# sara-nl/2D-VQ-AE-2

Hardware: AMD Instinct MI355X
Metric: patches/sec (VQAE.forward: encoder -> VQ -> decoder) (higher is better)
Workload: dtype f32; 1 GPU; BASELINE configs[1] (cfg B): batch 256/GPU of 256x256x3 fp32 -> 32x32 codes, K=256, D=128, full forward; global_batch=256, parallelism=patch-sharded x1

## Files before the change

### 2d-vq-ae-2_amd/csrc/conv_wino43.hip

```cpp
#include "kernels.h"
#include "mfma.h"

namespace {

using namespace vqae;

struct W43K {
    const float* __restrict__ t1;
    const float* __restrict__ U;
    const float* __restrict__ w3;
    const float* __restrict__ w1n;
    float* xio;
    float* y2;
    const float* __restrict__ Us;
    const float* __restrict__ w3s;
    const float* __restrict__ w1ns;
    int H, M;
    float act_a, act_b, t_scale, t_b4, n_b1a, n_b1b, n_b2a, n_b2b;
};

template <int C_> struct W43Cfg {
    static constexpr int C = C_;
    static constexpr int W = C >= 128 ? 32 : 64;
    static constexpr int NT = C == 256 ? 512 : 256;
    static constexpr int NWV = NT / 64;
    static constexpr int NS = C / 32;
    static constexpr int TG = NWV / NS;
    static constexpr int TILES = 16 * TG;
    static constexpr int TC = W / 4;
    static constexpr int PXH = 4 * W;
    static constexpr int C4 = C / 4;
    static constexpr int RP = NT / C4;
    static constexpr int LDT = C + 4;
    static constexpr int KG = C / 16;
    static constexpr int KS = C / 8;
    static constexpr int NI = 2;
    static constexpr int WN = C / (32 * NI);
    static constexpr int MI = PXH / ((NWV / WN) * 32);
    static constexpr int V_BYTES = 6 * TILES * LDT * 4, T_BYTES = PXH * LDT * 4;
    static constexpr int LDS_BYTES = V_BYTES > T_BYTES ? V_BYTES : T_BYTES;
    static constexpr int LDVB = 3 * C + 8, KC = C / 32, KS2 = C / 16;
    static constexpr int VS_BYTES = 6 * TILES * LDVB * 2;
    static constexpr int LDS_SPLIT = VS_BYTES > T_BYTES ? VS_BYTES : T_BYTES;
    static_assert(TILES == 2 * TC && RP == TC && PXH / RP == 16 && MI * NI == 4, "geometry");
};
constexpr int EARLY = 1;
constexpr int RD = 4;
constexpr int NRES0 = 4;
constexpr int RT = 3;

__device__ __forceinline__ void split3(const f32x4& v, bf16x4 (&h)[3]) {
    h[0] = __builtin_convertvector(v, bf16x4);
    const f32x4 r1 = v - __builtin_convertvector(h[0], f32x4);
    h[1] = __builtin_convertvector(r1, bf16x4);
    const f32x4 r2 = r1 - __builtin_convertvector(h[1], f32x4);
    h[2] = __builtin_convertvector(r2, bf16x4);
}
__device__ __forceinline__ bf16x8 as_bf8(const f32x4& v) { return __builtin_bit_cast(bf16x8, v); }

__device__ __forceinline__ f32x4 fma4(const f32x4& a, float s, const f32x4& c) {
    return __builtin_elementwise_fma(a, f32x4{s, s, s, s}, c);
}

__device__ __forceinline__ f32x4 ldg(const float* sbase, unsigned voff_bytes) {
    return *reinterpret_cast<const f32x4*>(reinterpret_cast<const char*>(sbase) + voff_bytes);
}

template <int N> struct IC { static constexpr int value = N; };

template <int C, int TAIL, bool SPLIT>
__global__ __launch_bounds__((W43Cfg<C>::NT), (W43Cfg<C>::NT == 512 ? 1 : 2))
void wino43_trunk_kernel(const W43K p) {
    using K = W43Cfg<C>;
    constexpr int W = K::W, LDT = K::LDT, KG = K::KG, KS = K::KS, TILES = K::TILES, TC = K::TC, NS = K::NS, C4 = K::C4, RP = K::RP;
    constexpr int MI = K::MI, NI = K::NI, WN = K::WN;
    constexpr int LDVB = K::LDVB, KC = K::KC, KS2 = K::KS2;
    extern __shared__ __attribute__((aligned(16))) float lds[];
    const int tid = threadIdx.x;
    const int lane = tid & 63;
    const int wave = __builtin_amdgcn_readfirstlane(tid >> 6);
    const int li = lane & 15, q = lane >> 4;
    const int ns = wave % NS, tg = wave / NS;

    int tile_m;
    {
        const int nwg = gridDim.x, bid = blockIdx.x;
        const int qq = nwg >> 3, r = nwg & 7, xcd = bid & 7;
        tile_m = (xcd < r ? xcd * (qq + 1) : r * (qq + 1) + (xcd - r) * qq) + (bid >> 3);
    }
    const int tpi = p.H / 8;
    const int img = tile_m / tpi;
    const int row0 = 8 * (tile_m - img * tpi);
    const float* const xim = p.t1 + (int64_t)img * p.H * W * C;

    const int cg = tid % C4, tj = tid / C4;
    unsigned coff[6];
    int roff[2][6];
#pragma unroll
    for (int j = 0; j < 6; ++j) coff[j] = (unsigned)((((4 * tj - 1 + j) & (W - 1)) * C + 4 * cg) * 4);
#pragma unroll
    for (int s = 0; s < 2; ++s)
#pragma unroll
        for (int i = 0; i < 6; ++i) {
            int r = row0 + 4 * s - 1 + i;
            r = r < 0 ? r + p.H : (r >= p.H ? r - p.H : r);
            roff[s][i] = r * W * C;
        }

    f32x4 d[2][4][2];
    f32x4 w[6];
    auto issue = [&](auto kind_c, int k) __attribute__((always_inline)) {
        constexpr int KIND = decltype(kind_c)::value;
        const int s = k / 3, cp = k % 3, bf = k & 1;
#pragma unroll
        for (int i = 0; i < (KIND == 1 ? 4 : 3); ++i) {
            const int row = KIND == 0 ? 2 * i : (KIND == 5 ? 2 * i + 1 : i + 1);
#pragma unroll
            for (int jj = 0; jj < 2; ++jj) d[bf][i][jj] = ldg(xim + roff[s][row], coff[2 * cp + jj]);
        }
    };
    auto combine = [&](auto kind_c, int k, float c1, float c2, float c3) __attribute__((always_inline)) {
        constexpr int KIND = decltype(kind_c)::value;
        const int cp = k % 3, bf = k & 1;
#pragma unroll
        for (int jj = 0; jj < 2; ++jj) {
            if (KIND == 1) w[2 * cp + jj] = fma4(d[bf][0][jj], c1, fma4(d[bf][1][jj], c2, fma4(d[bf][2][jj], c3, d[bf][3][jj])));
            else w[2 * cp + jj] = fma4(d[bf][0][jj], 4.f, fma4(d[bf][1][jj], -5.f, d[bf][2][jj]));
        }
    };
    auto columns = [&](int s) __attribute__((always_inline)) {
        float* const dst = lds + (s * TC + tj) * LDT + 4 * cg;
        __bf16* const dsb = reinterpret_cast<__bf16*>(lds) + (s * TC + tj) * LDVB + 4 * cg;
        auto put = [&](int nu, const f32x4& v) __attribute__((always_inline)) {
            if constexpr (SPLIT) {
                bf16x4 h[3];
                split3(v, h);
#pragma unroll
                for (int pl = 0; pl < 3; ++pl) *reinterpret_cast<bf16x4*>(dsb + nu * TILES * LDVB + pl * C) = h[pl];
            } else {
                *reinterpret_cast<f32x4*>(dst + nu * TILES * LDT) = v;
            }
        };
        const f32x4 t1 = fma4(w[2], -4.f, w[4]), t2 = fma4(w[1], -4.f, w[3]);
        const f32x4 t3 = w[4] - w[2], t4 = w[3] - w[1];
        put(0, fma4(w[0], 4.f, fma4(w[2], -5.f, w[4])));
        put(1, t1 + t2);
        put(2, t1 - t2);
        put(3, fma4(t4, 2.f, t3));
        put(4, fma4(t4, -2.f, t3));
        put(5, fma4(w[1], 4.f, fma4(w[3], -5.f, w[5])));
    };

    const float* const ub = p.U + ns * (KG * 512);
    const float* const ubs = p.Us + ns * (KC * 1536);
    const __bf16* const vbs = reinterpret_cast<const __bf16*>(lds) + (16 * tg + li) * LDVB + 8 * q;
    const unsigned wl = 16u * lane;
    const float* const bfrag = lds + (16 * tg + li) * LDT + 4 * q;

    f32x4 Y[4][4][2];
#pragma unroll
    for (int a = 0; a < 4; ++a)
#pragma unroll
        for (int b = 0; b < 4; ++b) { Y[a][b][0] = f32x4{0.f, 0.f, 0.f, 0.f}; Y[a][b][1] = f32x4{0.f, 0.f, 0.f, 0.f}; }

    auto pass = [&](auto kind_c, auto next_c, int xi, float c1, float c2, float c3, float a1, float a2, float a3) __attribute__((always_inline)) {
        constexpr int KIND = decltype(kind_c)::value;
        constexpr int NEXT = decltype(next_c)::value;
        __builtin_amdgcn_sched_barrier(0);
#pragma unroll
        for (int j = 0; j < 6; ++j) asm volatile("" : "+v"(coff[j]));
        if (EARLY < 1) issue(kind_c, 0);
        if (EARLY < 2) issue(kind_c, 1);
#pragma unroll
        for (int k = 0; k < 6; ++k) {
            combine(kind_c, k, c1, c2, c3);
            if (k % 3 == 2) columns(k / 3);
            if (k + 2 < 6) issue(kind_c, k + 2);
        }
        __builtin_amdgcn_sched_barrier(0);
        f32x4 Z[4][2];
        f32x4 acc[2][2];
        auto fold_nu = [&](int nu) __attribute__((always_inline)) {
#pragma unroll
            for (int bl = 0; bl < 2; ++bl) {
                if (nu == 0) Z[0][bl] = Z[0][bl] + acc[0][bl];
                if (nu == 2) {
                    const f32x4 sm = acc[1][bl] + acc[0][bl], df = acc[1][bl] - acc[0][bl];
                    Z[0][bl] = Z[0][bl] + sm; Z[2][bl] = Z[2][bl] + sm;
                    Z[1][bl] = Z[1][bl] + df; Z[3][bl] = Z[3][bl] + df;
                }
                if (nu == 4) {
                    const f32x4 sm = acc[1][bl] + acc[0][bl], df = acc[1][bl] - acc[0][bl];
                    Z[0][bl] = Z[0][bl] + sm; Z[2][bl] = fma4(sm, 4.f, Z[2][bl]);
                    Z[1][bl] = fma4(df, 2.f, Z[1][bl]); Z[3][bl] = fma4(df, 8.f, Z[3][bl]);
                }
                if (nu == 5) Z[3][bl] = Z[3][bl] + acc[1][bl];
            }
            if (nu == 0 || nu == 2 || nu == 4)
                asm volatile("" : "+v"(Z[0][0]), "+v"(Z[0][1]), "+v"(Z[1][0]), "+v"(Z[1][1]), "+v"(Z[2][0]), "+v"(Z[2][1]), "+v"(Z[3][0]), "+v"(Z[3][1]));
        };
        if constexpr (SPLIT) {
            int64_t uoff = (int64_t)xi * 6 * (3 * C * C / 2);
            asm volatile("" : "+s"(uoff));
            const float* const ux = ubs + uoff;
#define WS(s, bl, pl) (((s) / KC) * (3 * C * C / 2) + 1536 * ((s) % KC) + 256 * (3 * (bl) + (pl)))
#define VB(s, pl) (*reinterpret_cast<const bf16x8*>(vbs + ((s) / KC) * TILES * LDVB + (pl) * C + 32 * ((s) % KC)))
            f32x4 w0[2][2], w1[2], w2[2];
#pragma unroll
            for (int bl = 0; bl < 2; ++bl) {
                w0[0][bl] = ldg(ux + WS(0, bl, 0), wl);
                w1[bl] = ldg(ux + WS(0, bl, 1), wl);
                w2[bl] = ldg(ux + WS(0, bl, 2), wl);
                w0[1][bl] = ldg(ux + WS(1, bl, 0), wl);
            }
            lds_barrier();
#pragma unroll
            for (int b = 0; b < 4; ++b) { Z[b][0] = f32x4{0.f, 0.f, 0.f, 0.f}; Z[b][1] = f32x4{0.f, 0.f, 0.f, 0.f}; }
            bf16x8 vb0 = VB(0, 0), vb1 = VB(0, 1), vb2 = VB(0, 2);
#pragma unroll
            for (int nu = 0; nu < 6; ++nu) {
                const int st = nu & 1;
                acc[st][0] = f32x4{0.f, 0.f, 0.f, 0.f};
                acc[st][1] = f32x4{0.f, 0.f, 0.f, 0.f};
#pragma unroll
                for (int kc = 0; kc < KC; ++kc) {
                    const int s = KC * nu + kc, sl = s & 1;
                    const bool nxt = s + 1 < 6 * KC;
#define MM(wa, vb) for (int bl = 0; bl < 2; ++bl) acc[st][bl] = __builtin_amdgcn_mfma_f32_16x16x32_bf16(as_bf8(wa[bl]), vb, acc[st][bl], 0, 0, 0)
                    MM(w1, vb1);
                    MM(w1, vb0);
                    if (nxt) for (int bl = 0; bl < 2; ++bl) w1[bl] = ldg(ux + WS(s + 1, bl, 1), wl);
                    MM(w2, vb0);
                    if (nxt) for (int bl = 0; bl < 2; ++bl) w2[bl] = ldg(ux + WS(s + 1, bl, 2), wl);
                    MM(w0[sl], vb2);
                    if (nxt) vb2 = VB(s + 1, 2);
                    MM(w0[sl], vb1);
                    if (nxt) vb1 = VB(s + 1, 1);
                    MM(w0[sl], vb0);
                    if (s + 2 < 6 * KC) for (int bl = 0; bl < 2; ++bl) w0[sl][bl] = ldg(ux + WS(s + 2, bl, 0), wl);
                    if (nxt) vb0 = VB(s + 1, 0);
#undef MM
                    __builtin_amdgcn_sched_barrier(0);
                }
                fold_nu(nu);
            }
#undef WS
#undef VB
        } else {
            int64_t uoff = (int64_t)xi * 6 * (C * C);
            asm volatile("" : "+s"(uoff));
            const float* const ux = ub + uoff;
#define WB(s) (((s) / KG) * (C * C) + 512 * ((s) % KG))
            f32x4 wq[RD][2];
#pragma unroll
            for (int s = 0; s < RD; ++s) {
                wq[s][0] = ldg(ux + WB(s), wl);
                wq[s][1] = ldg(ux + WB(s) + 256, wl);
            }
            lds_barrier();
#pragma unroll
            for (int b = 0; b < 4; ++b) { Z[b][0] = f32x4{0.f, 0.f, 0.f, 0.f}; Z[b][1] = f32x4{0.f, 0.f, 0.f, 0.f}; }
            f32x4 bq[2];
            bq[0] = *reinterpret_cast<const f32x4*>(bfrag);
#pragma unroll
            for (int nu = 0; nu < 6; ++nu) {
                const int st = nu & 1;
                acc[st][0] = f32x4{0.f, 0.f, 0.f, 0.f};
                acc[st][1] = f32x4{0.f, 0.f, 0.f, 0.f};
#pragma unroll
                for (int kg = 0; kg < KG; ++kg) {
                    const int s = KG * nu + kg;
                    if (s + 1 < 6 * KG)
                        bq[(s + 1) & 1] = *reinterpret_cast<const f32x4*>(bfrag + ((s + 1) / KG) * TILES * LDT + 16 * ((s + 1) % KG));
                    const f32x4 wa = wq[s % RD][0], wb = wq[s % RD][1];
                    if (s + RD < 6 * KG) {
                        wq[s % RD][0] = ldg(ux + WB(s + RD), wl);
                        wq[s % RD][1] = ldg(ux + WB(s + RD) + 256, wl);
                    }
#pragma unroll
                    for (int j = 0; j < 4; ++j) {
                        acc[st][0] = __builtin_amdgcn_mfma_f32_16x16x4f32(wa[j], bq[s & 1][j], acc[st][0], 0, 0, 0);
                        acc[st][1] = __builtin_amdgcn_mfma_f32_16x16x4f32(wb[j], bq[s & 1][j], acc[st][1], 0, 0, 0);
                    }
                    __builtin_amdgcn_sched_barrier(0);
                }
                fold_nu(nu);
            }
#undef WB
        }
        __builtin_amdgcn_sched_barrier(0);
        if constexpr (NEXT == 9) {
#pragma unroll
            for (int k = 0; k < EARLY; ++k)
#pragma unroll
                for (int i = 0; i < 4; ++i) {
                    const int ro = xi < 4 ? roff[0][i + 1] : roff[0][i < 3 ? 2 * i + 1 : 5];
#pragma unroll
                    for (int jj = 0; jj < 2; ++jj) d[k & 1][i][jj] = ldg(xim + ro, coff[2 * k + jj]);
                }
        } else {
            if constexpr (NEXT >= 0 && EARLY >= 1) issue(next_c, 0);
            if constexpr (NEXT >= 0 && EARLY >= 2) issue(next_c, 1);
        }
#pragma unroll
        for (int b = 0; b < 4; ++b)
#pragma unroll
            for (int bl = 0; bl < 2; ++bl) {
                if (KIND == 0) Y[0][b][bl] = Y[0][b][bl] + Z[b][bl];
                else if (KIND == 5) Y[3][b][bl] = Y[3][b][bl] + Z[b][bl];
                else {
                    Y[0][b][bl] = Y[0][b][bl] + Z[b][bl];
                    Y[1][b][bl] = fma4(Z[b][bl], a1, Y[1][b][bl]);
                    Y[2][b][bl] = fma4(Z[b][bl], a2, Y[2][b][bl]);
                    Y[3][b][bl] = fma4(Z[b][bl], a3, Y[3][b][bl]);
                }
            }
        lds_barrier();
    };

    if (EARLY >= 1) issue(IC<0>{}, 0);
    if (EARLY >= 2) issue(IC<0>{}, 1);
    pass(IC<0>{}, IC<1>{}, 0, 0.f, 0.f, 0.f, 0.f, 0.f, 0.f);
#pragma unroll 1
    for (int xi = 1; xi <= 4; ++xi) {
        const float sg = (xi & 1) ? 1.f : -1.f;
        const bool lo = xi <= 2;
        const float c1 = lo ? -4.f * sg : -2.f * sg, c2 = lo ? -4.f : -1.f, c3 = lo ? sg : 2.f * sg;
        const float a1 = lo ? sg : 2.f * sg, a2 = lo ? 1.f : 4.f, a3 = lo ? sg : 8.f * sg;
        pass(IC<1>{}, IC<9>{}, xi, c1, c2, c3, a1, a2, a3);
    }
    pass(IC<5>{}, IC<-1>{}, 5, 0.f, 0.f, 0.f, 0.f, 0.f, 0.f);

    float* const T = lds;
    const int li32 = lane & 31, hh = lane >> 5;
    const int wm = wave / WN, wn = wave % WN;
    const int tj0 = tj;
    float* const trow = T + tj0 * LDT + 4 * cg;
    const int ty = (16 * tg + li) / TC, tx = (16 * tg + li) % TC;
    f32x4 bt[RT][NI];
    f32x4 bs0[2][NI], bs1[NI], bs2[NI];
    auto tail_prefetch = [&](const float* __restrict__ wsrc) __attribute__((always_inline)) {
        if constexpr (SPLIT) {
            const float* b0 = wsrc + (wn * NI) * (KS2 * 768);
#pragma unroll
            for (int ni = 0; ni < NI; ++ni) {
                bs0[0][ni] = ldg(b0 + ni * (KS2 * 768), wl);
                bs1[ni] = ldg(b0 + ni * (KS2 * 768) + 256, wl);
                bs2[ni] = ldg(b0 + ni * (KS2 * 768) + 512, wl);
                bs0[1][ni] = ldg(b0 + ni * (KS2 * 768) + 768, wl);
            }
            return;
        }
        const float* b0 = wsrc + (wn * NI) * (KS * 256);
#pragma unroll
        for (int u = 0; u < RT; ++u)
#pragma unroll
            for (int ni = 0; ni < NI; ++ni) bt[u][ni] = ldg(b0 + ni * (KS * 256) + 256 * u, wl);
    };
    f32x16 acc[MI][NI];
    auto gemm_tail_split = [&](const float* __restrict__ wsrc) __attribute__((always_inline)) {
        const float* a0 = T + (wm * MI * 32 + li32) * LDT + 8 * hh;
        const float* b0 = wsrc + (wn * NI) * (KS2 * 768);
#pragma unroll
        for (int ks = 0; ks < KS2; ++ks) {
            const int sl = ks & 1;
            bf16x8 x[MI][3];
#pragma unroll
            for (int mi = 0; mi < MI; ++mi) {
                bf16x4 lo[3], hi[3];
                split3(*reinterpret_cast<const f32x4*>(a0 + mi * 32 * LDT + 16 * ks), lo);
                split3(*reinterpret_cast<const f32x4*>(a0 + mi * 32 * LDT + 16 * ks + 4), hi);
#pragma unroll
                for (int pl = 0; pl < 3; ++pl) x[mi][pl] = __builtin_shufflevector(lo[pl], hi[pl], 0, 1, 2, 3, 4, 5, 6, 7);
            }
#define MM(wa, pb) for (int mi = 0; mi < MI; ++mi) for (int ni = 0; ni < NI; ++ni) \
                acc[mi][ni] = __builtin_amdgcn_mfma_f32_32x32x16_bf16(as_bf8(wa[ni]), x[mi][pb], acc[mi][ni], 0, 0, 0)
#define RELOAD(dst, k, pl) for (int ni = 0; ni < NI; ++ni) dst[ni] = ldg(b0 + ni * (KS2 * 768) + 768 * (k) + 256 * (pl), wl)
            MM(bs1, 1);
            MM(bs1, 0);
            if (ks + 1 < KS2) RELOAD(bs1, ks + 1, 1);
            MM(bs2, 0);
            if (ks + 1 < KS2) RELOAD(bs2, ks + 1, 2);
            MM(bs0[sl], 2);
            MM(bs0[sl], 1);
            MM(bs0[sl], 0);
            if (ks + 2 < KS2) RELOAD(bs0[sl], ks + 2, 0);
#undef MM
#undef RELOAD
            __builtin_amdgcn_sched_barrier(0);
        }
    };
    auto gemm_tail = [&](const float* __restrict__ wsrc) __attribute__((always_inline)) {
#pragma unroll
        for (int mi = 0; mi < MI; ++mi)
#pragma unroll
            for (int ni = 0; ni < NI; ++ni)
#pragma unroll
                for (int r = 0; r < 16; ++r) acc[mi][ni][r] = 0.f;
        if constexpr (SPLIT) {
            gemm_tail_split(wsrc);
            return;
        }
        const float* a0 = T + (wm * MI * 32 + li32) * LDT + 4 * hh;
        const float* b0 = wsrc + (wn * NI) * (KS * 256);
        f32x4 a[2][MI];
#pragma unroll
        for (int mi = 0; mi < MI; ++mi) a[0][mi] = *reinterpret_cast<const f32x4*>(a0 + mi * 32 * LDT);
#pragma unroll
        for (int ks = 0; ks < KS; ++ks) {
            if (ks + 1 < KS) {
#pragma unroll
                for (int mi = 0; mi < MI; ++mi) a[(ks + 1) & 1][mi] = *reinterpret_cast<const f32x4*>(a0 + mi * 32 * LDT + 8 * (ks + 1));
            }
            f32x4 bc[NI];
#pragma unroll
            for (int ni = 0; ni < NI; ++ni) bc[ni] = bt[ks % RT][ni];
            if (ks + RT < KS) {
#pragma unroll
                for (int ni = 0; ni < NI; ++ni) bt[ks % RT][ni] = ldg(b0 + ni * (KS * 256) + 256 * (ks + RT), wl);
            }
#pragma unroll
            for (int r = 0; r < 4; ++r)
#pragma unroll
                for (int mi = 0; mi < MI; ++mi)
#pragma unroll
                    for (int ni = 0; ni < NI; ++ni)
                        acc[mi][ni] = __builtin_amdgcn_mfma_f32_32x32x2f32(bc[ni][r], a[ks & 1][mi][r], acc[mi][ni], 0, 0, 0);
            __builtin_amdgcn_sched_barrier(0);
        }
    };
    auto acc_to_lds = [&]() __attribute__((always_inline)) {
#pragma unroll
        for (int ni = 0; ni < NI; ++ni)
#pragma unroll
            for (int mi = 0; mi < MI; ++mi)
#pragma unroll
                for (int g = 0; g < 4; ++g) {
                    f32x4 o;
#pragma unroll
                    for (int e = 0; e < 4; ++e) o[e] = acc[mi][ni][4 * g + e];
                    *reinterpret_cast<f32x4*>(T + (wm * MI * 32 + mi * 32 + li32) * LDT + (wn * NI + ni) * 32 + 8 * g + 4 * hh) = o;
                }
    };

#pragma unroll
    for (int hf = 0; hf < 2; ++hf) {
#pragma unroll
        for (int a2 = 0; a2 < 2; ++a2)
#pragma unroll
            for (int b = 0; b < 4; ++b)
#pragma unroll
                for (int bl = 0; bl < 2; ++bl) {
                    f32x4 o;
#pragma unroll
                    for (int e = 0; e < 4; ++e) o[e] = elu_act(Y[2 * hf + a2][b][bl][e] + p.act_a) + p.act_b;
                    *reinterpret_cast<f32x4*>(T + ((2 * ty + a2) * W + 4 * tx + b) * LDT + 32 * ns + 16 * bl + 4 * q) = o;
                }
        tail_prefetch(SPLIT ? p.w3s : p.w3);
        const int64_t pixb = ((int64_t)img * p.H + row0 + 2 * hf) * W + tj0;
        float* xr[4];
#pragma unroll
        for (int r = 0; r < 4; ++r) xr[r] = p.xio + (pixb + (int64_t)(4 * (r >> 1) + (r & 1)) * W) * C + 4 * cg;
        f32x4 res[16];
#pragma unroll
        for (int i = 0; i < (hf == 0 ? NRES0 : 16); ++i) res[i] = __builtin_nontemporal_load(reinterpret_cast<const f32x4*>(xr[(RP * i) / W] + ((RP * i) % W) * C));
        lds_barrier();
        gemm_tail(SPLIT ? p.w3s : p.w3);
        if (hf == 0) {
#pragma unroll
            for (int i = NRES0; i < 16; ++i) res[i] = __builtin_nontemporal_load(reinterpret_cast<const f32x4*>(xr[(RP * i) / W] + ((RP * i) % W) * C));
        }
        if (TAIL == 2) tail_prefetch(SPLIT ? p.w1ns : p.w1n);
        lds_barrier();
        acc_to_lds();
        lds_barrier();
#pragma unroll
        for (int i = 0; i < 16; ++i) {
            f32x4 t = *reinterpret_cast<const f32x4*>(trow + RP * i * LDT);
            t = t * p.t_scale;
            t = t + p.t_b4;
            t = t + res[i];
            __builtin_nontemporal_store(t, reinterpret_cast<f32x4*>(xr[(RP * i) / W] + ((RP * i) % W) * C));
            if (TAIL == 2) {
#pragma unroll
                for (int e = 0; e < 4; ++e) t[e] = elu_act(t[e] + p.n_b1a) + p.n_b1b;
                *reinterpret_cast<f32x4*>(trow + RP * i * LDT) = t;
            }
        }
        if constexpr (TAIL == 2) {
            lds_barrier();
            gemm_tail(SPLIT ? p.w1ns : p.w1n);
            lds_barrier();
            acc_to_lds();
            lds_barrier();
            float* const y0 = p.y2 + (xr[0] - p.xio);
#pragma unroll
            for (int i = 0; i < 16; ++i) {
                f32x4 t = *reinterpret_cast<const f32x4*>(trow + RP * i * LDT);
#pragma unroll
                for (int e = 0; e < 4; ++e) t[e] = elu_act(t[e] + p.n_b2a) + p.n_b2b;
                const int r = (RP * i) / W;
                __builtin_nontemporal_store(t, reinterpret_cast<f32x4*>(y0 + ((4 * (r >> 1) + (r & 1)) * W + (RP * i) % W) * C));
            }
        }
        if (hf == 0) lds_barrier();
    }
}

__device__ void wino43_u(const float* __restrict__ w, int64_t i, double (&u)[36]) {
    const double G[6][3] = {{0.25, 0, 0}, {-1.0 / 6, -1.0 / 6, -1.0 / 6}, {-1.0 / 6, 1.0 / 6, -1.0 / 6},
                            {1.0 / 24, 1.0 / 12, 1.0 / 6}, {1.0 / 24, -1.0 / 12, 1.0 / 6}, {0, 0, 1}};
    double g[3][3], t[6][3];
    for (int a = 0; a < 3; ++a)
        for (int b = 0; b < 3; ++b) g[a][b] = (double)w[i * 9 + a * 3 + b];
    for (int x = 0; x < 6; ++x)
        for (int b = 0; b < 3; ++b) t[x][b] = G[x][0] * g[0][b] + G[x][1] * g[1][b] + G[x][2] * g[2][b];
    for (int x = 0; x < 6; ++x)
        for (int y = 0; y < 6; ++y) u[x * 6 + y] = t[x][0] * G[y][0] + t[x][1] * G[y][1] + t[x][2] * G[y][2];
}

__global__ void wino43_weight_kernel(const float* __restrict__ w, int c, float* __restrict__ U) {
    const int i = blockIdx.x * blockDim.x + threadIdx.x;
    if (i >= c * c) return;
    double u[36];
    wino43_u(w, i, u);
    const int n = i / c, k = i % c;
    const int64_t fo = ((((int64_t)(n >> 5) * (c / 16) + (k >> 4)) * 2 + ((n >> 4) & 1)) * 64 + ((k >> 2) & 3) * 16 + (n & 15)) * 4 + (k & 3);
    const int64_t cc = (int64_t)c * c;
    for (int x = 0; x < 36; ++x) U[x * cc + fo] = (float)u[x];
}

__device__ void split3_f64(double v, __bf16 (&h)[3]) {
    for (int pl = 0; pl < 3; ++pl) {
        h[pl] = (__bf16)(float)v;
        v -= (double)(float)h[pl];
    }
}

__global__ void wino43_split_weight_kernel(const float* __restrict__ w, int c, __bf16* __restrict__ U) {
    const int i = blockIdx.x * blockDim.x + threadIdx.x;
    if (i >= c * c) return;
    double u[36];
    wino43_u(w, i, u);
    const int n = i / c, k = i % c;
    const int64_t fo = (((int64_t)(n >> 5) * (c / 32) + (k >> 5)) * 2 + ((n >> 4) & 1)) * 3 * 512 + (((k >> 3) & 3) * 16 + (n & 15)) * 8 + (k & 7);
    const int64_t cc = (int64_t)c * c;
    for (int x = 0; x < 36; ++x) {
        __bf16 h[3];
        split3_f64(u[x], h);
        for (int pl = 0; pl < 3; ++pl) U[x * 3 * cc + fo + pl * 512] = h[pl];
    }
}

__global__ void split_1x1_kernel(const float* __restrict__ w, int c, __bf16* __restrict__ out) {
    const int i = blockIdx.x * blockDim.x + threadIdx.x;
    if (i >= c * c) return;
    const int n = i / c, k = i % c;
    __bf16 h[3];
    split3_f64((double)w[i], h);
    const int64_t fo = ((int64_t)(n >> 5) * (c / 16) + (k >> 4)) * 3 * 512 + (((k >> 3) & 1) * 32 + (n & 31)) * 8 + (k & 7);
    for (int pl = 0; pl < 3; ++pl) out[fo + pl * 512] = h[pl];
}

}

namespace vqae {

bool wino43_channels(int c) { return c == 256 || c == 128 || c == 64; }

bool wino43_supported(int c, int h, int w, int dtype) {
    return dtype == VQAE_DT_F32 && wino43_channels(c) && w == (c == 64 ? 64 : 32) && h >= 8 && h % 8 == 0;
}
bool wino43_enabled() { return env_int("VQAE_WINO43", 1) != 0; }

size_t wino43_weight_floats(int c) { return (size_t)36 * c * c; }

bool wino43_split_supported(int c) { return c == 128; }
size_t wino43_split_weight_bytes(int c) { return (size_t)36 * c * c * 3 * 2; }
size_t split_1x1_bytes(int c) { return (size_t)c * c * 3 * 2; }

int wino43_split_weight(const float* w_oihw_dev, int c, void* U_dev, hipStream_t stream) {
    VQAE_REQUIRE(wino43_split_supported(c), VQAE_ERR_UNSUPPORTED, "wino43_split_weight: C = %d", c);
    wino43_split_weight_kernel<<<(unsigned)ceil_div(c * c, 256), 256, 0, stream>>>(w_oihw_dev, c, (__bf16*)U_dev);
    VQAE_LAUNCH_CHECK();
    return VQAE_OK;
}

int split_1x1_weight(const float* w_packed_dev, int c, void* out_dev, hipStream_t stream) {
    VQAE_REQUIRE(wino43_split_supported(c), VQAE_ERR_UNSUPPORTED, "split_1x1_weight: C = %d", c);
    split_1x1_kernel<<<(unsigned)ceil_div(c * c, 256), 256, 0, stream>>>(w_packed_dev, c, (__bf16*)out_dev);
    VQAE_LAUNCH_CHECK();
    return VQAE_OK;
}

int wino43_transform_weight(const float* w_oihw_dev, int c, float* U_dev, hipStream_t stream) {
    VQAE_REQUIRE(wino43_channels(c), VQAE_ERR_UNSUPPORTED, "wino43_transform_weight: C = %d", c);
    wino43_weight_kernel<<<(unsigned)ceil_div(c * c, 256), 256, 0, stream>>>(w_oihw_dev, c, U_dev);
    VQAE_LAUNCH_CHECK();
    return VQAE_OK;
}

template <int C, bool SPLIT>
static int launch_w43(W43K& k, int64_t M, bool chain, hipStream_t stream) {
    using K = W43Cfg<C>;
    constexpr int lds = SPLIT ? K::LDS_SPLIT : K::LDS_BYTES;
    if (int rc = set_max_dynamic_lds((const void*)wino43_trunk_kernel<C, 1, SPLIT>, lds)) return rc;
    if (int rc = set_max_dynamic_lds((const void*)wino43_trunk_kernel<C, 2, SPLIT>, lds)) return rc;
    const unsigned grid = (unsigned)(M / (8 * K::W));
    const double flops = 2.0 * (double)M * C * (2.25 * C + C + (chain ? C : 0));
    ProfScope prof(C >= 128 ? PROF_CONV3X3_TRUNK : PROF_NONE, stream, flops);
    if (chain) wino43_trunk_kernel<C, 2, SPLIT><<<grid, K::NT, lds, stream>>>(k);
    else wino43_trunk_kernel<C, 1, SPLIT><<<grid, K::NT, lds, stream>>>(k);
    prof.done();
    VQAE_LAUNCH_CHECK();
    return VQAE_OK;
}

int wino43_trunk_tail(const float* t1, const float* U, const float* w3, float act_a, float act_b, float t_scale, float t_b4,
                      float* xio, const NextConv1& next, int batch, int h, int w, int c, hipStream_t stream,
                      const void* Us, const void* w3s) {
    if (batch == 0) return VQAE_OK;
    const float* w1n = (const float*)next.w1;
    float* t1_next = (float*)next.t1_next;
    VQAE_REQUIRE(t1 && U && w3 && xio && (!w1n || t1_next), VQAE_ERR_INVALID, "wino43_trunk_tail: null pointer");
    VQAE_REQUIRE(wino43_supported(c, h, w, VQAE_DT_F32), VQAE_ERR_UNSUPPORTED, "wino43_trunk_tail: C = %d, H = %d, W = %d", c, h, w);
    const int64_t M = (int64_t)batch * h * w;
    VQAE_REQUIRE(M < (1ll << 31) - 1024, VQAE_ERR_UNSUPPORTED, "wino43_trunk_tail: too many pixels");
    W43K k;
    memset(&k, 0, sizeof(k));
    k.t1 = t1; k.U = U; k.w3 = w3; k.w1n = w1n; k.xio = xio; k.y2 = t1_next;
    k.H = h; k.M = (int)M;
    k.act_a = act_a; k.act_b = act_b; k.t_scale = t_scale; k.t_b4 = t_b4;
    k.n_b1a = next.b1a; k.n_b1b = next.b1b; k.n_b2a = next.b2a; k.n_b2b = next.b2b;
    if (Us) {
        VQAE_REQUIRE(wino43_split_supported(c) && w3s && (!w1n || next.w1s), VQAE_ERR_INVALID, "wino43_trunk_tail: split form needs C = 128 and its three weights");
        k.Us = (const float*)Us; k.w3s = (const float*)w3s; k.w1ns = (const float*)next.w1s;
        return launch_w43<128, true>(k, M, w1n != nullptr, stream);
    }
    switch (c) {
        case 256: return launch_w43<256, false>(k, M, w1n != nullptr, stream);
        case 128: return launch_w43<128, false>(k, M, w1n != nullptr, stream);
        default: return launch_w43<64, false>(k, M, w1n != nullptr, stream);
    }
}

}
```

Measured before the change: 4252 patches/s.

## Add wide two-band split Winograd trunk kernel for C=128

Adds a WIDE variant of the split-bf16 Winograd F(4,3) trunk kernel for C=128 that processes two 8-row bands per workgroup with 512 threads. Each wave pair splits the weight planes, and the 6 transform slices are divided into low/high LDS regions. The aim is to load each weight fragment once and reuse it across twice as many tiles, and to halve the number of workgroups. In exchange it needs more LDS per block, has more complex addressing, and launches fewer blocks, which can hurt occupancy and the tail wave.

```diff
diff --git a/2d-vq-ae-2_amd/csrc/conv_wino43.hip b/2d-vq-ae-2_amd/csrc/conv_wino43.hip
--- a/2d-vq-ae-2_amd/csrc/conv_wino43.hip
+++ b/2d-vq-ae-2_amd/csrc/conv_wino43.hip
@@ -19,16 +19,19 @@
     float act_a, act_b, t_scale, t_b4, n_b1a, n_b1b, n_b2a, n_b2b;
 };
 
-template <int C_> struct W43Cfg {
+template <int C_, bool WIDE_ = false> struct W43Cfg {
     static constexpr int C = C_;
+    static constexpr bool WIDE = WIDE_;
+    static constexpr int BANDS = WIDE ? 2 : 1;
+    static constexpr int ROWS = 8 * BANDS;
     static constexpr int W = C >= 128 ? 32 : 64;
-    static constexpr int NT = C == 256 ? 512 : 256;
+    static constexpr int NT = (C == 256 || WIDE) ? 512 : 256;
     static constexpr int NWV = NT / 64;
     static constexpr int NS = C / 32;
     static constexpr int TG = NWV / NS;
     static constexpr int TILES = 16 * TG;
     static constexpr int TC = W / 4;
-    static constexpr int PXH = 4 * W;
+    static constexpr int PXH = 4 * W * BANDS;
     static constexpr int C4 = C / 4;
     static constexpr int RP = NT / C4;
     static constexpr int LDT = C + 4;
@@ -42,7 +45,8 @@
     static constexpr int LDVB = 3 * C + 8, KC = C / 32, KS2 = C / 16;
     static constexpr int VS_BYTES = 6 * TILES * LDVB * 2;
     static constexpr int LDS_SPLIT = VS_BYTES > T_BYTES ? VS_BYTES : T_BYTES;
-    static_assert(TILES == 2 * TC && RP == TC && PXH / RP == 16 && MI * NI == 4, "geometry");
+    static_assert(TILES == 2 * TC * BANDS && RP == TC * BANDS && PXH / RP == 16 && MI * NI == 4, "geometry");
+    static_assert(!WIDE || C == 128, "the wide form serves C = 128");
 };
 constexpr int EARLY = 1;
 constexpr int RD = 4;
@@ -68,10 +72,13 @@
 
 template <int N> struct IC { static constexpr int value = N; };
 
-template <int C, int TAIL, bool SPLIT>
-__global__ __launch_bounds__((W43Cfg<C>::NT), (W43Cfg<C>::NT == 512 ? 1 : 2))
+constexpr int tail_row(int r) { return 8 * (r >> 2) + 4 * ((r >> 1) & 1) + (r & 1); }
+
+template <int C, int TAIL, bool SPLIT, bool WIDE = false>
+__global__ __launch_bounds__((W43Cfg<C, WIDE>::NT), (W43Cfg<C, WIDE>::NT == 512 ? 1 : 2))
 void wino43_trunk_kernel(const W43K p) {
-    using K = W43Cfg<C>;
+    using K = W43Cfg<C, WIDE>;
+    static_assert(!WIDE || SPLIT, "the wide form is a split form");
     constexpr int W = K::W, LDT = K::LDT, KG = K::KG, KS = K::KS, TILES = K::TILES, TC = K::TC, NS = K::NS, C4 = K::C4, RP = K::RP;
     constexpr int MI = K::MI, NI = K::NI, WN = K::WN;
     constexpr int LDVB = K::LDVB, KC = K::KC, KS2 = K::KS2;
@@ -80,7 +87,7 @@
     const int lane = tid & 63;
     const int wave = __builtin_amdgcn_readfirstlane(tid >> 6);
     const int li = lane & 15, q = lane >> 4;
-    const int ns = wave % NS, tg = wave / NS;
+    const int ns = WIDE ? wave >> 1 : wave % NS, tg = WIDE ? 0 : wave / NS;
 
     int tile_m;
     {
@@ -88,21 +95,22 @@
         const int qq = nwg >> 3, r = nwg & 7, xcd = bid & 7;
         tile_m = (xcd < r ? xcd * (qq + 1) : r * (qq + 1) + (xcd - r) * qq) + (bid >> 3);
     }
-    const int tpi = p.H / 8;
+    const int tpi = p.H / K::ROWS;
     const int img = tile_m / tpi;
-    const int row0 = 8 * (tile_m - img * tpi);
+    const int row0 = K::ROWS * (tile_m - img * tpi);
     const float* const xim = p.t1 + (int64_t)img * p.H * W * C;
 
     const int cg = tid % C4, tj = tid / C4;
+    const int tjc = WIDE ? tj & (TC - 1) : tj, band = WIDE ? wave >> 2 : 0;
     unsigned coff[6];
     int roff[2][6];
 #pragma unroll
-    for (int j = 0; j < 6; ++j) coff[j] = (unsigned)((((4 * tj - 1 + j) & (W - 1)) * C + 4 * cg) * 4);
+    for (int j = 0; j < 6; ++j) coff[j] = (unsigned)((((4 * tjc - 1 + j) & (W - 1)) * C + 4 * cg) * 4);
 #pragma unroll
     for (int s = 0; s < 2; ++s)
 #pragma unroll
         for (int i = 0; i < 6; ++i) {
-            int r = row0 + 4 * s - 1 + i;
+            int r = row0 + 8 * band + 4 * s - 1 + i;
             r = r < 0 ? r + p.H : (r >= p.H ? r - p.H : r);
             roff[s][i] = r * W * C;
         }
@@ -129,14 +137,19 @@
         }
     };
     auto columns = [&](int s) __attribute__((always_inline)) {
-        float* const dst = lds + (s * TC + tj) * LDT + 4 * cg;
-        __bf16* const dsb = reinterpret_cast<__bf16*>(lds) + (s * TC + tj) * LDVB + 4 * cg;
+        float* const dst = lds + (16 * band + s * TC + tjc) * LDT + 4 * cg;
+        __bf16* const dsb = reinterpret_cast<__bf16*>(lds) + (16 * band + s * TC + tjc) * LDVB + 4 * cg;
+        int vhi = 3 * TILES * LDVB;
+        if constexpr (WIDE) asm volatile("" : "+v"(vhi));
         auto put = [&](int nu, const f32x4& v) __attribute__((always_inline)) {
             if constexpr (SPLIT) {
                 bf16x4 h[3];
                 split3(v, h);
 #pragma unroll
-                for (int pl = 0; pl < 3; ++pl) *reinterpret_cast<bf16x4*>(dsb + nu * TILES * LDVB + pl * C) = h[pl];
+                for (int pl = 0; pl < 3; ++pl) {
+                    if (WIDE && nu >= 3) *reinterpret_cast<bf16x4*>(dsb + vhi + (nu - 3) * TILES * LDVB + pl * C) = h[pl];
+                    else *reinterpret_cast<bf16x4*>(dsb + nu * TILES * LDVB + pl * C) = h[pl];
+                }
             } else {
                 *reinterpret_cast<f32x4*>(dst + nu * TILES * LDT) = v;
             }
@@ -152,7 +165,7 @@
     };
 
     const float* const ub = p.U + ns * (KG * 512);
-    const float* const ubs = p.Us + ns * (KC * 1536);
+    const float* const ubs = p.Us + ns * (KC * 1536) + (WIDE ? 768 * (wave & 1) : 0);
     const __bf16* const vbs = reinterpret_cast<const __bf16*>(lds) + (16 * tg + li) * LDVB + 8 * q;
     const unsigned wl = 16u * lane;
     const float* const bfrag = lds + (16 * tg + li) * LDT + 4 * q;
@@ -199,7 +212,58 @@
             if (nu == 0 || nu == 2 || nu == 4)
                 asm volatile("" : "+v"(Z[0][0]), "+v"(Z[0][1]), "+v"(Z[1][0]), "+v"(Z[1][1]), "+v"(Z[2][0]), "+v"(Z[2][1]), "+v"(Z[3][0]), "+v"(Z[3][1]));
         };
-        if constexpr (SPLIT) {
+        if constexpr (WIDE) {
+            int64_t uoff = (int64_t)xi * 6 * (3 * C * C / 2);
+            asm volatile("" : "+s"(uoff));
+            const float* const ux = ubs + uoff;
+#define WS(s, pl) (((s) / KC) * (3 * C * C / 2) + 1536 * ((s) % KC) + 256 * (pl))
+            int vhi = 3 * TILES * LDVB;
+            asm volatile("" : "+v"(vhi));
+            const __bf16* const vbh = vbs + vhi;
+#define VB(s, g, pl) (*reinterpret_cast<const bf16x8*>(((s) / KC >= 3 ? vbh - 3 * TILES * LDVB : vbs) + ((s) / KC) * TILES * LDVB + (g) * 16 * LDVB + (pl) * C + 32 * ((s) % KC)))
+            f32x4 w0[2], w1[2], w2[2];
+            w1[0] = ldg(ux + WS(0, 1), wl);
+            w2[0] = ldg(ux + WS(0, 2), wl);
+            w0[0] = ldg(ux + WS(0, 0), wl);
+            w1[1] = ldg(ux + WS(1, 1), wl);
+            w2[1] = ldg(ux + WS(1, 2), wl);
+            w0[1] = ldg(ux + WS(1, 0), wl);
+            lds_barrier();
+#pragma unroll
+            for (int b = 0; b < 4; ++b) { Z[b][0] = f32x4{0.f, 0.f, 0.f, 0.f}; Z[b][1] = f32x4{0.f, 0.f, 0.f, 0.f}; }
+            bf16x8 vb0[2], vb1[2], vb2[2];
+#pragma unroll
+            for (int g = 0; g < 2; ++g) { vb0[g] = VB(0, g, 0); vb1[g] = VB(0, g, 1); vb2[g] = VB(0, g, 2); }
+#pragma unroll
+            for (int nu = 0; nu < 6; ++nu) {
+                const int st = nu & 1;
+                acc[st][0] = f32x4{0.f, 0.f, 0.f, 0.f};
+                acc[st][1] = f32x4{0.f, 0.f, 0.f, 0.f};
+#pragma unroll
+                for (int kc = 0; kc < KC; ++kc) {
+                    const int s = KC * nu + kc, sl = s & 1;
+                    const bool nxt = s + 1 < 6 * KC;
+#define MM(wa, vb) for (int g = 0; g < 2; ++g) acc[st][g] = __builtin_amdgcn_mfma_f32_16x16x32_bf16(as_bf8(wa), vb[g], acc[st][g], 0, 0, 0)
+                    MM(w1[sl], vb1);
+                    MM(w1[sl], vb0);
+                    if (s + 2 < 6 * KC) w1[sl] = ldg(ux + WS(s + 2, 1), wl);
+                    MM(w2[sl], vb0);
+                    if (s + 2 < 6 * KC) w2[sl] = ldg(ux + WS(s + 2, 2), wl);
+                    MM(w0[sl], vb2);
+                    if (nxt) for (int g = 0; g < 2; ++g) vb2[g] = VB(s + 1, g, 2);
+                    MM(w0[sl], vb1);
+                    if (nxt) for (int g = 0; g < 2; ++g) vb1[g] = VB(s + 1, g, 1);
+                    MM(w0[sl], vb0);
+                    if (s + 2 < 6 * KC) w0[sl] = ldg(ux + WS(s + 2, 0), wl);
+                    if (nxt) for (int g = 0; g < 2; ++g) vb0[g] = VB(s + 1, g, 0);
+#undef MM
+                    __builtin_amdgcn_sched_barrier(0);
+                }
+                fold_nu(nu);
+            }
+#undef WS
+#undef VB
+        } else if constexpr (SPLIT) {
             int64_t uoff = (int64_t)xi * 6 * (3 * C * C / 2);
             asm volatile("" : "+s"(uoff));
             const float* const ux = ubs + uoff;
@@ -335,7 +399,7 @@
     const int li32 = lane & 31, hh = lane >> 5;
     const int wm = wave / WN, wn = wave % WN;
     const int tj0 = tj;
-    float* const trow = T + tj0 * LDT + 4 * cg;
+    [[maybe_unused]] float* const trow = WIDE ? nullptr : T + tj0 * LDT + 4 * cg;
     const int ty = (16 * tg + li) / TC, tx = (16 * tg + li) % TC;
     f32x4 bt[RT][NI];
     f32x4 bs0[2][NI], bs1[NI], bs2[NI];
@@ -445,6 +509,14 @@
 
 #pragma unroll
     for (int hf = 0; hf < 2; ++hf) {
+        int tbo = (2 * ty * W + 4 * tx) * LDT + 16 * wave + 4 * q, tro = tj0 * LDT + 4 * cg;
+        if constexpr (WIDE) asm volatile("" : "+v"(tbo), "+v"(tro));
+        int tbo1 = tbo + 4 * W * LDT, tro1 = tro + 8 * RP * LDT;
+        if constexpr (WIDE) asm volatile("" : "+v"(tbo1), "+v"(tro1));
+        auto tr = [&](int i) __attribute__((always_inline)) {
+            if constexpr (WIDE) return reinterpret_cast<f32x4*>(T + (i < 8 ? tro + RP * i * LDT : tro1 + RP * (i - 8) * LDT));
+            else return reinterpret_cast<f32x4*>(trow + RP * i * LDT);
+        };
 #pragma unroll
         for (int a2 = 0; a2 < 2; ++a2)
 #pragma unroll
@@ -454,21 +526,40 @@
                     f32x4 o;
 #pragma unroll
                     for (int e = 0; e < 4; ++e) o[e] = elu_act(Y[2 * hf + a2][b][bl][e] + p.act_a) + p.act_b;
-                    *reinterpret_cast<f32x4*>(T + ((2 * ty + a2) * W + 4 * tx + b) * LDT + 32 * ns + 16 * bl + 4 * q) = o;
+                    if constexpr (WIDE) *reinterpret_cast<f32x4*>(T + (bl ? tbo1 : tbo) + (a2 * W + b) * LDT) = o;
+                    else *reinterpret_cast<f32x4*>(T + ((2 * ty + a2) * W + 4 * tx + b) * LDT + 32 * ns + 16 * bl + 4 * q) = o;
                 }
         tail_prefetch(SPLIT ? p.w3s : p.w3);
-        const int64_t pixb = ((int64_t)img * p.H + row0 + 2 * hf) * W + tj0;
-        float* xr[4];
-#pragma unroll
-        for (int r = 0; r < 4; ++r) xr[r] = p.xio + (pixb + (int64_t)(4 * (r >> 1) + (r & 1)) * W) * C + 4 * cg;
+        [[maybe_unused]] float* xr[WIDE ? 1 : K::PXH / W];
+        [[maybe_unused]] int64_t xu = 0;
+        [[maybe_unused]] unsigned xvo = 0;
+        if constexpr (WIDE) {
+            xu = (((int64_t)img * p.H + row0 + 2 * hf) * W) * C;
+            xvo = (unsigned)((tj0 * C + 4 * cg) * 4);
+            asm volatile("" : "+v"(xvo));
+        } else {
+            const int64_t pixb = ((int64_t)img * p.H + row0 + 2 * hf) * W + tj0;
+#pragma unroll
+            for (int r = 0; r < K::PXH / W; ++r) xr[r] = p.xio + (pixb + (int64_t)(4 * (r >> 1) + (r & 1)) * W) * C + 4 * cg;
+        }
+        auto xp = [&](float* base, int i) __attribute__((always_inline)) {
+            const int r = (RP * i) / W;
+            if constexpr (WIDE) {
+                int64_t ro = xu + (tail_row(r) * W + (RP * i) % W) * C;
+                asm volatile("" : "+s"(ro));
+                return reinterpret_cast<f32x4*>(reinterpret_cast<char*>(base + ro) + xvo);
+            } else {
+                return reinterpret_cast<f32x4*>(xr[r] + ((RP * i) % W) * C);
+            }
+        };
         f32x4 res[16];
 #pragma unroll
-        for (int i = 0; i < (hf == 0 ? NRES0 : 16); ++i) res[i] = __builtin_nontemporal_load(reinterpret_cast<const f32x4*>(xr[(RP * i) / W] + ((RP * i) % W) * C));
+        for (int i = 0; i < (hf == 0 ? NRES0 : 16); ++i) res[i] = __builtin_nontemporal_load(xp(p.xio, i));
         lds_barrier();
         gemm_tail(SPLIT ? p.w3s : p.w3);
         if (hf == 0) {
 #pragma unroll
-            for (int i = NRES0; i < 16; ++i) res[i] = __builtin_nontemporal_load(reinterpret_cast<const f32x4*>(xr[(RP * i) / W] + ((RP * i) % W) * C));
+            for (int i = NRES0; i < 16; ++i) res[i] = __builtin_nontemporal_load(xp(p.xio, i));
         }
         if (TAIL == 2) tail_prefetch(SPLIT ? p.w1ns : p.w1n);
         lds_barrier();
@@ -476,15 +567,15 @@
         lds_barrier();
 #pragma unroll
         for (int i = 0; i < 16; ++i) {
-            f32x4 t = *reinterpret_cast<const f32x4*>(trow + RP * i * LDT);
+            f32x4 t = *tr(i);
             t = t * p.t_scale;
             t = t + p.t_b4;
             t = t + res[i];
-            __builtin_nontemporal_store(t, reinterpret_cast<f32x4*>(xr[(RP * i) / W] + ((RP * i) % W) * C));
+            __builtin_nontemporal_store(t, xp(p.xio, i));
             if (TAIL == 2) {
 #pragma unroll
                 for (int e = 0; e < 4; ++e) t[e] = elu_act(t[e] + p.n_b1a) + p.n_b1b;
-                *reinterpret_cast<f32x4*>(trow + RP * i * LDT) = t;
+                *tr(i) = t;
             }
         }
         if constexpr (TAIL == 2) {
@@ -493,14 +584,16 @@
             lds_barrier();
             acc_to_lds();
             lds_barrier();
-            float* const y0 = p.y2 + (xr[0] - p.xio);
+            [[maybe_unused]] float* y0 = nullptr;
+            if constexpr (!WIDE) y0 = p.y2 + (xr[0] - p.xio);
 #pragma unroll
             for (int i = 0; i < 16; ++i) {
-                f32x4 t = *reinterpret_cast<const f32x4*>(trow + RP * i * LDT);
+                f32x4 t = *tr(i);
 #pragma unroll
                 for (int e = 0; e < 4; ++e) t[e] = elu_act(t[e] + p.n_b2a) + p.n_b2b;
                 const int r = (RP * i) / W;
-                __builtin_nontemporal_store(t, reinterpret_cast<f32x4*>(y0 + ((4 * (r >> 1) + (r & 1)) * W + (RP * i) % W) * C));
+                if constexpr (WIDE) __builtin_nontemporal_store(t, xp(p.y2, i));
+                else __builtin_nontemporal_store(t, reinterpret_cast<f32x4*>(y0 + ((4 * (r >> 1) + (r & 1)) * W + (RP * i) % W) * C));
             }
         }
         if (hf == 0) lds_barrier();
@@ -600,17 +693,17 @@
     return VQAE_OK;
 }
 
-template <int C, bool SPLIT>
+template <int C, bool SPLIT, bool WIDE = false>
 static int launch_w43(W43K& k, int64_t M, bool chain, hipStream_t stream) {
-    using K = W43Cfg<C>;
+    using K = W43Cfg<C, WIDE>;
     constexpr int lds = SPLIT ? K::LDS_SPLIT : K::LDS_BYTES;
-    if (int rc = set_max_dynamic_lds((const void*)wino43_trunk_kernel<C, 1, SPLIT>, lds)) return rc;
-    if (int rc = set_max_dynamic_lds((const void*)wino43_trunk_kernel<C, 2, SPLIT>, lds)) return rc;
-    const unsigned grid = (unsigned)(M / (8 * K::W));
+    if (int rc = set_max_dynamic_lds((const void*)wino43_trunk_kernel<C, 1, SPLIT, WIDE>, lds)) return rc;
+    if (int rc = set_max_dynamic_lds((const void*)wino43_trunk_kernel<C, 2, SPLIT, WIDE>, lds)) return rc;
+    const unsigned grid = (unsigned)(M / (K::ROWS * K::W));
     const double flops = 2.0 * (double)M * C * (2.25 * C + C + (chain ? C : 0));
     ProfScope prof(C >= 128 ? PROF_CONV3X3_TRUNK : PROF_NONE, stream, flops);
-    if (chain) wino43_trunk_kernel<C, 2, SPLIT><<<grid, K::NT, lds, stream>>>(k);
-    else wino43_trunk_kernel<C, 1, SPLIT><<<grid, K::NT, lds, stream>>>(k);
+    if (chain) wino43_trunk_kernel<C, 2, SPLIT, WIDE><<<grid, K::NT, lds, stream>>>(k);
+    else wino43_trunk_kernel<C, 1, SPLIT, WIDE><<<grid, K::NT, lds, stream>>>(k);
     prof.done();
     VQAE_LAUNCH_CHECK();
     return VQAE_OK;
@@ -635,6 +728,7 @@
     if (Us) {
         VQAE_REQUIRE(wino43_split_supported(c) && w3s && (!w1n || next.w1s), VQAE_ERR_INVALID, "wino43_trunk_tail: split form needs C = 128 and its three weights");
         k.Us = (const float*)Us; k.w3s = (const float*)w3s; k.w1ns = (const float*)next.w1s;
+        if (h % 16 == 0) return launch_w43<128, true, true>(k, M, w1n != nullptr, stream);
         return launch_w43<128, true>(k, M, w1n != nullptr, stream);
     }
     switch (c) {
```

Measured after the change: 4482 patches/s (median of 6 runs). 1.05x the previous value.
